# mauriceqch/pcc_geo_cnn_v2

Hardware: AMD Instinct MI355X
Metric: voxel_blocks_64cubed_per_sec_encode_decode (higher is better)
Workload: dtype f32

## Files before the change

include/pcc_geo.h:

```cpp
#ifndef PCC_GEO_H
#define PCC_GEO_H

#include <stddef.h>
#include <stdint.h>

#ifdef __cplusplus
extern "C" {
#endif

#define PCC_ABI_VERSION 4

#define PCC_OK 0
#define PCC_ERR_ARG (-1)
#define PCC_ERR_HIP (-2)
#define PCC_ERR_NOGPU (-3)
#define PCC_ERR_SPACE (-4)
#define PCC_ERR_CORRUPT (-5)

typedef struct pcc_ctx pcc_ctx;

int pcc_abi_version(void);
const char* pcc_last_error(void);
int pcc_ctx_create(int device, pcc_ctx** out);
int pcc_ctx_destroy(pcc_ctx* ctx);
int pcc_ctx_num_cu(pcc_ctx* ctx);

#define PCC_KERNEL_FAMILY 6
#define PCC_NUM_NO_SPLIT 0x1
#define PCC_NUM_NO_SPLIT_DIRECT 0x2
#define PCC_NUM_NO_SPLIT_TR2 0x4
#define PCC_NUM_NO_WINOGRAD 0x8
#define PCC_NUM_NO_WINOGRAD32 0x10
#define PCC_NUM_NO_WINOGRAD64 0x20
#define PCC_NUM_WINO_PER_GROUP 0x40
#define PCC_NUM_NO_TR2M 0x80
#define PCC_NUM_TR2M 0x100
#define PCC_NUM_TR2_OLD 0x200
#define PCC_NUM_SPLIT_MFMA16 0x400
#define PCC_NUM_SPLIT_MFMA32 0x800
#define PCC_NUM_SPLIT_TILE8 0x1000
#define PCC_NUM_P16 0x2000
#define PCC_NUM_NO_F16S 0x4000
#define PCC_NUM_COUT1_T16 0x8000
int pcc_ctx_get_numerics(pcc_ctx* ctx, uint32_t* family, uint32_t* switches);
int pcc_ctx_set_numerics(pcc_ctx* ctx, uint32_t switches);

#define PCC_CONV_BIAS 1
#define PCC_CONV_RELU 2
#define PCC_CONV_ADD 4
#define PCC_CONV_CLIP01 8
#define PCC_CONV_F16 16

#define PCC_CONV_IN16 32
#define PCC_CONV_OUT16 64
#define PCC_CONV_RES16 128

#define PCC_IMPL_AUTO 0
#define PCC_IMPL_GENERIC 1
#define PCC_IMPL_MFMA 2
#define PCC_IMPL_WINOGRAD 3
#define PCC_IMPL_SPLIT 4

typedef struct {
    int32_t N, D, H, W;
    int32_t Cin, Cout;
    int32_t k;
    int32_t stride;
    int32_t transposed;
    int32_t flags;
    int32_t impl;
    int32_t out_cstride;
    int32_t out_coffset;
} pcc_conv_desc;

int pcc_conv_out_dims(const pcc_conv_desc* d, int32_t* OD, int32_t* OH, int32_t* OW);
int pcc_conv_mfma_supported(const pcc_conv_desc* d);
size_t pcc_conv_packed_floats(const pcc_conv_desc* d);
int pcc_conv_pack_weights(const pcc_conv_desc* d, const float* w_keras_host, float* packed_host);
int pcc_conv_kernel_family(pcc_ctx* ctx, const pcc_conv_desc* d, char* buf, int32_t cap);
int pcc_conv3d(pcc_ctx* ctx, const pcc_conv_desc* d, const float* in, const float* w,
               const float* w_packed, const float* bias, const float* residual, float* out,
               void* stream);

#define PCC_NET_ANALYSIS_V1 0
#define PCC_NET_SYNTHESIS_V1 1
#define PCC_NET_ANALYSIS_V2 2
#define PCC_NET_SYNTHESIS_V2 3
#define PCC_NET_ANALYSIS_PROGRESSIVE_V2 4
#define PCC_NET_SYNTHESIS_PROGRESSIVE_V2 5
#define PCC_NET_HYPER_ANALYSIS 6
#define PCC_NET_HYPER_SYNTHESIS 7

int32_t pcc_network_num_layers(int32_t transform, int32_t filters);
int pcc_network_layer(int32_t transform, int32_t filters, int32_t layer, pcc_conv_desc* d, int32_t* residual_role);
size_t pcc_weights_blob_floats(int32_t transform, int32_t filters);
int pcc_weights_pack(int32_t transform, int32_t filters, const float* const* kernels, const float* const* biases,
                     float* blob_host);
int pcc_weights_upload(pcc_ctx* ctx, int32_t transform, int32_t filters, const float* const* kernels,
                       const float* const* biases, float* blob_device, void* stream);
size_t pcc_network_workspace_bytes(int32_t transform, int32_t filters, int32_t N, int32_t D, int32_t H, int32_t W);
int pcc_network_out_dims(int32_t transform, int32_t filters, int32_t D, int32_t H, int32_t W, int32_t* OD, int32_t* OH,
                         int32_t* OW, int32_t* OC);
typedef struct {
    pcc_conv_desc desc;
    int32_t record_amax;
} pcc_layer_plan;
int pcc_network_plan(const pcc_conv_desc* layers, const int32_t* roles, int32_t n, int32_t N, int32_t D, int32_t H, int32_t W,
                     int32_t layer_flags, int32_t final_flags, uint32_t numerics, pcc_layer_plan* plan, int32_t* any_amax);
int pcc_network_forward(pcc_ctx* ctx, int32_t transform, int32_t filters, const float* blob, const float* x, int32_t N,
                        int32_t D, int32_t H, int32_t W, float* y, void* workspace, size_t workspace_bytes,
                        int32_t layer_flags, int32_t final_flags, void* stream);
int pcc_network_forward_analysis(pcc_ctx* ctx, int32_t transform, int32_t filters, const float* blob, const float* x,
                                 int32_t N, int32_t D, int32_t H, int32_t W, float* y, void* workspace,
                                 size_t workspace_bytes, int32_t layer_flags, int32_t final_flags, void* stream);
int pcc_network_forward_synthesis(pcc_ctx* ctx, int32_t transform, int32_t filters, const float* blob, const float* x,
                                  int32_t N, int32_t D, int32_t H, int32_t W, float* y, void* workspace,
                                  size_t workspace_bytes, int32_t layer_flags, int32_t final_flags, void* stream);
int pcc_network_forward_hyper_a(pcc_ctx* ctx, int32_t transform, int32_t filters, const float* blob, const float* x,
                                int32_t N, int32_t D, int32_t H, int32_t W, float* y, void* workspace,
                                size_t workspace_bytes, int32_t layer_flags, int32_t final_flags, void* stream);
int pcc_network_forward_hyper_s(pcc_ctx* ctx, int32_t transform, int32_t filters, const float* blob, const float* x,
                                int32_t N, int32_t D, int32_t H, int32_t W, float* y, void* workspace,
                                size_t workspace_bytes, int32_t layer_flags, int32_t final_flags, void* stream);

typedef struct {
    int32_t version;
    int32_t filters;
    int32_t analysis, synthesis;
    const float* w_analysis;
    const float* w_synthesis;
    const float* w_hyper_analysis;
    const float* w_hyper_synthesis;
// ... 304 lines not shown
```

pcc_geo_cnn_v2_amd/_lib.py:

```python
import ctypes as C
import os

_HERE = os.path.dirname(os.path.abspath(__file__))
LIB_PATH = os.environ.get('PCC_GEO_LIB', os.path.join(_HERE, 'libpcc_geo_hip.so'))

PCC_CONV_BIAS, PCC_CONV_RELU, PCC_CONV_ADD, PCC_CONV_CLIP01, PCC_CONV_F16 = 1, 2, 4, 8, 16
PCC_CONV_IN16, PCC_CONV_OUT16, PCC_CONV_RES16 = 32, 64, 128
PCC_IMPL_AUTO, PCC_IMPL_GENERIC, PCC_IMPL_MFMA, PCC_IMPL_WINOGRAD, PCC_IMPL_SPLIT = 0, 1, 2, 3, 4
PCC_ROUND_FLOOR_HALF, PCC_ROUND_HALF_EVEN = 0, 1
PCC_ANCHOR_NO_CONTEXT, PCC_ANCHOR_HDR_WORDS = 1, 32
PCC_SURFACE_HDR_WORDS = 4
PCC_COLOR_HDR_WORDS = 72

EXPORTS = [
    'pcc_abi_version', 'pcc_last_error', 'pcc_ctx_create', 'pcc_ctx_destroy', 'pcc_ctx_num_cu', 'pcc_ctx_get_numerics', 'pcc_ctx_set_numerics',
    'pcc_conv_out_dims', 'pcc_conv_mfma_supported', 'pcc_conv_packed_floats', 'pcc_conv_pack_weights', 'pcc_conv_kernel_family',
    'pcc_conv3d', 'pcc_quantize', 'pcc_dequantize', 'pcc_scale_to_index', 'pcc_threshold_compact',
    'pcc_threshold_scratch_ints', 'pcc_voxelize', 'pcc_focal_loss', 'pcc_focal_scratch_floats',
    'pcc_symbols_tiles', 'pcc_symbols_pack', 'pcc_symbols_unpack', 'pcc_quantize_pack', 'pcc_index_pack', 'pcc_unpack_dequantize',
    'pcc_range_encode_batch', 'pcc_range_decode_batch', 'pcc_range_encode_batch_n', 'pcc_range_decode_batch_n', 'pcc_pmf_to_quantized_cdf',
    'pcc_d1_search_workspace_bytes', 'pcc_d1_threshold_stats', 'pcc_d12_search_workspace_bytes', 'pcc_d12_threshold_stats', 'pcc_octree_bucket',
    'pcc_d12_search_ties_chunk', 'pcc_d12_search_ties_workspace_bytes', 'pcc_d12_threshold_stats_ties',
    'pcc_network_num_layers', 'pcc_network_layer', 'pcc_weights_blob_floats', 'pcc_weights_pack', 'pcc_weights_upload',
    'pcc_network_workspace_bytes', 'pcc_network_out_dims', 'pcc_network_plan', 'pcc_network_forward', 'pcc_network_forward_analysis',
    'pcc_network_forward_synthesis', 'pcc_network_forward_hyper_a', 'pcc_network_forward_hyper_s',
    'pcc_codec_workspace_bytes', 'pcc_codec_encode', 'pcc_codec_decode_hyper', 'pcc_codec_decode_main',
    'pcc_profile_select', 'pcc_profile_read', 'pcc_normals_workspace_bytes', 'pcc_estimate_normals',
    'pcc_cloud_index_bytes', 'pcc_cloud_index_build', 'pcc_cloud_nearest', 'pcc_cloud_distortion_workspace_bytes', 'pcc_cloud_distortion',
    'pcc_cloud_distortion_ties_workspace_bytes', 'pcc_cloud_distortion_ties',
    'pcc_cloud_map_colors', 'pcc_cloud_color_workspace_bytes', 'pcc_cloud_color_distortion',
    'pcc_cloud_transfer_workspace_bytes', 'pcc_cloud_transfer_colors',
    'pcc_mesh_sample_workspace_bytes', 'pcc_mesh_to_points', 'pcc_render_workspace_bytes', 'pcc_render_points',
    'pcc_conv_wgrad_workspace_bytes', 'pcc_conv_wgrad_slices', 'pcc_conv3d_wgrad', 'pcc_relu_backward', 'pcc_focal_loss_grad', 'pcc_conv_repack_map',
    'pcc_conv_repack_weights_device',
    'pcc_histogram_limits', 'pcc_tensor_histogram_workspace_bytes', 'pcc_tensor_histogram_slices', 'pcc_tensor_histogram', 'pcc_occupancy_scores',
    'pcc_anchor_code_bits', 'pcc_anchor_decode_bits', 'pcc_anchor_encode', 'pcc_anchor_decoder_bytes', 'pcc_anchor_decoder_init',
    'pcc_anchor_decode_level', 'pcc_anchor_decoder_consumed', 'pcc_anchor_tree_capacity', 'pcc_anchor_tree_level_offset',
    'pcc_anchor_tree_workspace_bytes', 'pcc_anchor_tree', 'pcc_anchor_expand_workspace_bytes', 'pcc_anchor_expand', 'pcc_anchor_points',
    'pcc_surface_encode_vertices', 'pcc_surface_decode_vertices', 'pcc_surface_leaves_workspace_bytes', 'pcc_surface_leaves',
    'pcc_surface_edges_workspace_bytes', 'pcc_surface_edges', 'pcc_surface_vertices_workspace_bytes', 'pcc_surface_vertices',
    'pcc_surface_count_workspace_bytes', 'pcc_surface_count', 'pcc_surface_reconstruct_workspace_bytes', 'pcc_surface_reconstruct',
    'pcc_color_anchor_workspace_bytes', 'pcc_color_anchor_plan', 'pcc_color_anchor_forward', 'pcc_color_anchor_inverse',
    'pcc_color_anchor_encode', 'pcc_color_anchor_decode',
    'pcc_rans_stream_cap', 'pcc_rans_workspace_bytes', 'pcc_rans_check_strings', 'pcc_rans_encode_batch', 'pcc_rans_decode_batch',
    'pcc_occ_stream_cap', 'pcc_occ_workspace_bytes', 'pcc_occ_check_strings', 'pcc_occ_encode_batch', 'pcc_occ_decode_batch',
    'pcc_topk_workspace_bytes', 'pcc_topk_compact',
    'pcc_rank_levels_workspace_bytes', 'pcc_rank_levels', 'pcc_d1_count_stats', 'pcc_d12_count_stats',
    'pcc_d1_threshold_stats_hausdorff', 'pcc_d12_threshold_stats_hausdorff', 'pcc_d1_count_stats_hausdorff', 'pcc_d12_count_stats_hausdorff',
    'pcc_quantize_step_pack', 'pcc_index_pack_step', 'pcc_unpack_dequantize_step', 'pcc_rate_ladder',
]
ABI_VERSION = 4
PCC_NUM = dict(no_split=0x1, no_split_direct=0x2, no_split_tr2=0x4, no_winograd=0x8, no_winograd32=0x10, no_winograd64=0x20,
               wino_per_group=0x40, no_tr2m=0x80, tr2m=0x100, tr2_old=0x200, split_mfma16=0x400, split_mfma32=0x800, split_tile8=0x1000,
               p16=0x2000, no_f16s=0x4000, cout1_t16=0x8000)
PCC_ERR_ARG, PCC_ERR_HIP, PCC_ERR_NOGPU, PCC_ERR_SPACE, PCC_ERR_CORRUPT = -1, -2, -3, -4, -5
(PCC_NET_ANALYSIS_V1, PCC_NET_SYNTHESIS_V1, PCC_NET_ANALYSIS_V2, PCC_NET_SYNTHESIS_V2, PCC_NET_ANALYSIS_PROGRESSIVE_V2,
 PCC_NET_SYNTHESIS_PROGRESSIVE_V2, PCC_NET_HYPER_ANALYSIS, PCC_NET_HYPER_SYNTHESIS) = range(8)


class ConvDesc(C.Structure):
    _fields_ = [(n, C.c_int32) for n in ('N', 'D', 'H', 'W', 'Cin', 'Cout', 'k', 'stride', 'transposed',
                                         'flags', 'impl', 'out_cstride', 'out_coffset')]


class LayerPlan(C.Structure):
    _fields_ = [('desc', ConvDesc), ('record_amax', C.c_int32)]


class CdfTable(C.Structure):
    _fields_ = [('cdf', C.POINTER(C.c_int32)), ('cdf_size', C.POINTER(C.c_int32)), ('offset', C.POINTER(C.c_int32)),
                ('rows', C.c_int32), ('cdf_stride', C.c_int32), ('precision', C.c_int32),
                ('overflow_width', C.c_int32)]


class CodecDesc(C.Structure):
    _fields_ = [('version', C.c_int32), ('filters', C.c_int32), ('analysis', C.c_int32), ('synthesis', C.c_int32),
                ('w_analysis', C.c_void_p), ('w_synthesis', C.c_void_p), ('w_hyper_analysis', C.c_void_p),
                ('w_hyper_synthesis', C.c_void_p), ('medians', C.c_void_p), ('scale_table', C.c_void_p),
                ('scale_levels', C.c_int32), ('round_mode', C.c_int32)]


class SymbolSink(C.Structure):
    _fields_ = [('zsym', C.c_void_p), ('ysym', C.c_void_p), ('idx', C.c_void_p), ('zsym_tile_max', C.c_void_p),
                ('ysym_tile_max', C.c_void_p), ('sym_bytes', C.c_int32), ('idx_bytes', C.c_int32), ('channels_first', C.c_int32)]


HISTOGRAM_BUCKETS = 1551


class Histogram(C.Structure):
    _fields_ = [('counts', C.c_uint64 * HISTOGRAM_BUCKETS), ('num', C.c_uint64), ('nonfinite', C.c_uint64), ('min', C.c_double),
                ('max', C.c_double), ('sum', C.c_double), ('sum_squares', C.c_double)]


class Occupancy(C.Structure):
    _fields_ = [(n, C.c_uint64) for n in ('tp', 'tn', 'fp', 'fn', 'num_occupied')]


class PccError(RuntimeError):
    pass


_lib = None


def lib():
    global _lib
    if _lib is not None:
        return _lib
    import torch
    if not os.path.exists(LIB_PATH):
        raise PccError(f'{LIB_PATH} is missing: build it with `make -C pcc_geo_cnn_v2_amd/csrc` '
                       '(python -c "import __graft_entry__ as g; g.build()"). There is no CPU fallback.')
    L = C.CDLL(LIB_PATH)
    vp, i32, sz = C.c_void_p, C.c_int32, C.c_size_t
    L.pcc_abi_version.argtypes, L.pcc_abi_version.restype = [], C.c_int
    L.pcc_last_error.argtypes, L.pcc_last_error.restype = [], C.c_char_p
    L.pcc_ctx_create.argtypes = [C.c_int, C.POINTER(vp)]
    L.pcc_ctx_destroy.argtypes = [vp]
    L.pcc_ctx_num_cu.argtypes = [vp]
    L.pcc_ctx_get_numerics.argtypes = [vp, C.POINTER(C.c_uint32), C.POINTER(C.c_uint32)]
    L.pcc_ctx_set_numerics.argtypes = [vp, C.c_uint32]
    L.pcc_conv_out_dims.argtypes = [C.POINTER(ConvDesc), C.POINTER(i32), C.POINTER(i32), C.POINTER(i32)]
    L.pcc_conv_mfma_supported.argtypes = [C.POINTER(ConvDesc)]
    L.pcc_conv_packed_floats.argtypes = [C.POINTER(ConvDesc)]
    L.pcc_conv_packed_floats.restype = sz
    L.pcc_conv_kernel_family.argtypes = [vp, C.POINTER(ConvDesc), C.c_char_p, i32]
    L.pcc_conv_pack_weights.argtypes = [C.POINTER(ConvDesc), vp, vp]
    L.pcc_conv3d.argtypes = [vp, C.POINTER(ConvDesc), vp, vp, vp, vp, vp, vp, vp]
    L.pcc_quantize.argtypes = [vp, vp, vp, vp, vp, sz, i32, i32, vp]
    L.pcc_dequantize.argtypes = [vp, vp, vp, vp, sz, i32, vp]
    L.pcc_scale_to_index.argtypes = [vp, vp, vp, i32, vp, sz, vp]
    L.pcc_threshold_compact.argtypes = [vp, vp, i32, i32, i32, i32, vp, i32, vp, vp, C.c_int64, vp, vp]
    L.pcc_threshold_scratch_ints.argtypes = [i32, i32, i32, i32]
    L.pcc_threshold_scratch_ints.restype = sz
    L.pcc_voxelize.argtypes = [vp, vp, vp, C.c_int64, i32, i32, i32, i32, vp, vp]
    L.pcc_focal_loss.argtypes = [vp, vp, vp, sz, C.c_float, C.c_float, vp, vp, vp]
    L.pcc_focal_scratch_floats.argtypes, L.pcc_focal_scratch_floats.restype = [], sz
    L.pcc_range_encode_batch.argtypes = [C.POINTER(CdfTable), i32, vp, vp, i32, vp, vp, vp, vp, i32]
    L.pcc_range_decode_batch.argtypes = [C.POINTER(CdfTable), i32, vp, vp, vp, i32, vp, vp, i32]
    L.pcc_range_encode_batch_n.argtypes = [C.POINTER(CdfTable), i32, vp, i32, vp, i32, i32, vp, vp, vp, vp, i32]
    L.pcc_range_decode_batch_n.argtypes = [C.POINTER(CdfTable), i32, vp, vp, vp, i32, i32, vp, vp, i32, i32]
    L.pcc_pmf_to_quantized_cdf.argtypes = [vp, i32, i32, vp]
    L.pcc_d1_search_workspace_bytes.argtypes = [i32, i32, i32, i32]
    L.pcc_d1_search_workspace_bytes.restype = sz
    L.pcc_d1_threshold_stats.argtypes = [vp, vp, i32, i32, i32, i32, vp, i32, i32, vp, vp, C.c_int64, vp, vp, vp, vp, vp, vp]
    L.pcc_d12_search_workspace_bytes.argtypes = [i32, i32, i32, i32, C.c_int64]
    L.pcc_d12_search_workspace_bytes.restype = sz
    L.pcc_d12_threshold_stats.argtypes = [vp, vp, i32, i32, i32, i32, vp, i32, i32, vp, vp, vp, C.c_int64, vp, vp, vp, vp, vp, vp, vp, vp, vp, vp]
    L.pcc_d12_search_ties_chunk.argtypes = [i32, i32, i32, i32]
    L.pcc_d12_search_ties_chunk.restype = i32
    L.pcc_d12_search_ties_workspace_bytes.argtypes = [i32, i32, i32, i32, C.c_int64, C.c_int64]
    L.pcc_d12_search_ties_workspace_bytes.restype = sz
    L.pcc_d12_threshold_stats_ties.argtypes = [vp, vp, i32, i32, i32, i32, vp, i32, i32, vp, vp, vp, C.c_int64, vp, C.c_int64, vp, vp, vp, vp, vp, vp,
                                               vp, vp, vp, vp]
    L.pcc_normals_workspace_bytes.argtypes = [C.c_int64, i32]
    L.pcc_normals_workspace_bytes.restype = sz
    L.pcc_estimate_normals.argtypes = [vp, vp, C.c_int64, i32, vp, vp, vp, vp, vp]
    L.pcc_cloud_index_bytes.argtypes = [C.c_int64]
    L.pcc_cloud_index_bytes.restype = sz
    L.pcc_cloud_index_build.argtypes = [vp, vp, C.c_int64, vp, vp]
    L.pcc_cloud_nearest.argtypes = [vp, vp, C.c_int64, vp, C.c_int64, vp, vp, vp]
    L.pcc_cloud_distortion_workspace_bytes.argtypes = [C.c_int64, C.c_int64]
    L.pcc_cloud_distortion_workspace_bytes.restype = sz
    L.pcc_cloud_distortion.argtypes = [vp, vp, C.c_int64, vp, C.c_int64, vp, vp, vp, vp, vp, vp]
    L.pcc_cloud_distortion_ties_workspace_bytes.argtypes = [C.c_int64, C.c_int64, i32, C.c_int64]
    L.pcc_cloud_distortion_ties_workspace_bytes.restype = sz
    L.pcc_cloud_distortion_ties.argtypes = [vp, vp, C.c_int64, vp, C.c_int64, vp, i32, C.c_int64, vp, vp, vp, vp, vp, vp]
    L.pcc_cloud_map_colors.argtypes = [vp, vp, C.c_int64, vp, vp, C.c_int64, i32, vp, vp, vp]
    L.pcc_cloud_color_workspace_bytes.argtypes = [C.c_int64, C.c_int64]
    L.pcc_cloud_color_workspace_bytes.restype = sz
    L.pcc_cloud_color_distortion.argtypes = [vp, vp, C.c_int64, vp, vp, C.c_int64, vp, vp, vp, vp]
    L.pcc_cloud_transfer_workspace_bytes.argtypes = [C.c_int64, C.c_int64]
    L.pcc_cloud_transfer_workspace_bytes.restype = sz
    L.pcc_cloud_transfer_colors.argtypes = [vp, vp, C.c_int64, vp, vp, C.c_int64, vp, vp, vp, vp]
    L.pcc_mesh_sample_workspace_bytes.argtypes = [C.c_int64, C.c_int64]
    L.pcc_mesh_sample_workspace_bytes.restype = sz
    L.pcc_mesh_to_points.argtypes = [vp, vp, C.c_int64, vp, C.c_int64, C.c_int64, C.c_uint64, i32, vp, vp, vp, vp, vp]
    L.pcc_render_workspace_bytes.argtypes = [i32, i32]
    L.pcc_render_workspace_bytes.restype = sz
# ... 124 lines not shown
```

pcc_geo_cnn_v2_amd/csrc/common.h:

```cpp
#pragma once
#include <hip/hip_runtime.h>

#include <cstdarg>
#include <cstdio>

#include "../../include/pcc_geo.h"

struct pcc_ctx {
    int device;
    int num_cu;
    hipDeviceProp_t prop;
    void* profile = nullptr;
    void* scratch = nullptr;
    size_t scratch_bytes = 0;
    uint32_t numerics = 0;
    bool num(uint32_t bit) const { return (numerics & bit) != 0; }
    unsigned* amax = nullptr;
    int amax_cap = 0;
    void* summary_limits = nullptr;
};
int pcc_ctx_amax(pcc_ctx* ctx, int n, unsigned** ptr);
constexpr int PCC_AMAX_SLOTS = 64;
struct pcc_conv_ext { const unsigned* in_amax; unsigned* out_amax; bool out_recorded; };
#ifdef __HIPCC__
// ... 64 lines not shown
}
int pcc_conv3d_ext(pcc_ctx* ctx, const pcc_conv_desc* d, const float* in, const float* w, const float* w_packed, const float* bias,
                   const float* residual, float* out, pcc_conv_ext* ext, void* stream);
uint32_t* pcc_threshold_mask_of(int32_t* scratch, int32_t B, int32_t D);
int pcc_threshold_from_mask(pcc_ctx* ctx, int32_t B, int32_t D, int32_t H, int32_t W, float* xyz, int32_t* counts, int64_t cap,
                            int32_t* scratch, hipStream_t st);
bool pcc_wino_eligible(const pcc_conv_desc* d);
int pcc_conv_wino(pcc_ctx* ctx, const pcc_conv_desc* d, const float* in, const float* u_packed,
                  const float* bias, const float* residual, float* out, hipStream_t st);
bool pcc_tr2m_eligible(const pcc_conv_desc* d);
int pcc_conv_tr2m(pcc_ctx* ctx, const pcc_conv_desc* d, const float* in, const float* w_tr2g, const float* bias, float* out,
                  hipStream_t st);
size_t pcc_tr2m_bf16_packed_floats(int Cin, int Cout);
void pcc_tr2m_bf16_pack(int Cin, int Cout, const float* w_tr2g, float* out);
bool pcc_tr2m_bf16_covers(const pcc_conv_desc* d);
int pcc_conv_tr2m_bf16(pcc_ctx* ctx, const pcc_conv_desc* d, const float* in, const float* w_split, const float* bias, float* out,
                       pcc_conv_ext* ext, hipStream_t st);
constexpr int PCC_TR2M_F16S_TAIL = 64;
size_t pcc_tr2m_f16s_packed_floats(int Cin, int Cout);
void pcc_tr2m_f16s_pack(int Cin, int Cout, const float* w_tr2g, float* out);
int pcc_conv_tr2m_f16s(pcc_ctx* ctx, const pcc_conv_desc* d, const float* in, const float* w_f16s, const float* bias, float* out,
                       pcc_conv_ext* ext, hipStream_t st);
bool pcc_tr2m_f16_covers(const pcc_conv_desc* d);
int pcc_conv_tr2m_f16(pcc_ctx* ctx, const pcc_conv_desc* d, const float* in, const float* w_tr2g, const float* bias, void* out,
                      hipStream_t st);
bool pcc_f16_eligible(const pcc_conv_desc* d);
size_t pcc_f16_packed_bytes(int C);
void pcc_f16_pack(int C, const float* wlog, unsigned short* out);
int pcc_conv_f16(pcc_ctx* ctx, const pcc_conv_desc* d, const void* in, const void* w_packed, const float* bias,
                 const void* residual, void* out, bool out32, hipStream_t st);
constexpr int PCC_WINO_U_FLOATS = 48 * 64 * 4;
constexpr int PCC_WINO_UB_FLOATS = 48 * 2 * 64 * 4;
void pcc_wino_bf16_pack(int ngroups, const float* u_f32, float* out);
int pcc_conv_wino_bf16(pcc_ctx* ctx, const pcc_conv_desc* d, const float* in, const float* ub_packed, const float* bias,
                       const float* residual, float* out, hipStream_t st);
constexpr int PCC_WINO_UH_FLOATS = 64 * 776 / 4;
constexpr int PCC_WINO_UH_TAIL = 64;
bool pcc_wino_f16s_covers(const pcc_conv_desc* d);
void pcc_wino_f16s_pack(int ngroups, const float* u_f32, float* out);
int pcc_conv_wino_f16s(pcc_ctx* ctx, const pcc_conv_desc* d, const float* in, const float* uh_packed, const float* bias,
                       const float* residual, float* out, pcc_conv_ext* ext, hipStream_t st);
size_t pcc_split_packed_floats(int C);
void pcc_split_pack(int C, const float* wlog, float* out);
bool pcc_split_covers(const pcc_conv_desc* d);
bool pcc_tr2_split_covers(const pcc_conv_desc* d);
int pcc_conv_tr2_split(pcc_ctx* ctx, const pcc_conv_desc* d, const float* in, const float* w_split, const float* bias, float* out,
                       pcc_conv_ext* ext, hipStream_t st);
int pcc_conv_split(pcc_ctx* ctx, const pcc_conv_desc* d, bool mfma32, const float* in, const float* w_split, const float* bias,
                   const float* residual, float* out, hipStream_t st);
int pcc_conv_fwd(pcc_ctx* ctx, const pcc_conv_desc* d, const float* in, const float* w_packed, const float* bias, const float* residual,
                 float* out, int tx, hipStream_t st);
int pcc_conv_tr2(pcc_ctx* ctx, const pcc_conv_desc* d, const float* in, const float* w_packed, const float* bias, const float* residual,
                 float* out, int tx, hipStream_t st);
int pcc_conv_cin1(pcc_ctx* ctx, const pcc_conv_desc* d, const float* in, const float* w_packed, const float* bias, const float* residual,
                  float* out, pcc_conv_ext* ext, hipStream_t st);
int pcc_conv_cout1_mfma(pcc_ctx* ctx, const pcc_conv_desc* d, const float* in, const float* w_packed, const float* bias,
                        const float* residual, float* out, const pcc_thr_fuse* fuse, bool* fused, hipStream_t st);
int pcc_conv_cout1(pcc_ctx* ctx, const pcc_conv_desc* d, const float* in, const float* w_packed, const float* bias, const float* residual,
                   float* out, hipStream_t st);
#include <utility>
#include <vector>
inline int pcc_enable_big_lds(const void* kern, int lds_bytes) {
    if (lds_bytes <= 64 * 1024) return PCC_OK;
    static thread_local std::vector<std::pair<const void*, int>> done;
    int dev = 0;
    PCC_CHECK_HIP(hipGetDevice(&dev));
    for (const auto& e : done)
        if (e.first == kern && e.second == dev) return PCC_OK;
    PCC_CHECK_HIP(hipFuncSetAttribute(kern, hipFuncAttributeMaxDynamicSharedMemorySize, lds_bytes));
    done.emplace_back(kern, dev);
    return PCC_OK;
}

inline bool pcc_wino_channels(int cin, int cout) { return cin == cout && (cin == 16 || cin == 32 || cin == 64); }
```

pcc_geo_cnn_v2_amd/csrc/conv_route.hip:

```cpp
#include <cstdlib>

#include "common.h"

namespace {

enum Kind { K_NONE = 0, K_FWD, K_TR2, K_CIN1, K_COUT1, K_COUT1M };

struct Plan {
    Kind kind = K_NONE;
    int tx = 0;
    bool flip = false;
};

inline int base_w(const pcc_conv_desc* d) {
    if (d->transposed) return d->W;
    return pcc_same_out(d->W, d->stride);
}

static Plan make_plan(const pcc_conv_desc* d) {
    Plan p;
    if ((double)d->D * d->H * d->W * d->Cin * 4.0 >= 2147483648.0) return p;
    const bool out_vec_ok = d->out_cstride == 0 || (d->out_cstride % 4 == 0 && d->out_coffset % 4 == 0);
    const int k = d->k, s = d->stride;
    const bool even = (d->D % 2 == 0) && (d->H % 2 == 0) && (d->W % 2 == 0);
// ... 185 lines not shown
    PCC_REQUIRE(p.kind != K_NONE, "pcc_conv_pack_weights: shape not covered by the MFMA path");
    const Packed L = packed_layout(d, p.kind);
    const Taps Wf{d, w, p.flip};
    switch (p.kind) {
        case K_FWD: return pack_fwd(d, Wf, L, pk);
        case K_TR2: pack_tr2(d, Wf, L, pk); break;
        case K_CIN1: pack_cin1(d, Wf, pk); break;
        case K_COUT1M: pack_cout1m(Wf, pk); break;
        default: pack_cout1(d, Wf, pk);
    }
    return PCC_OK;
}

pcc_conv_family pcc_conv_route(const pcc_conv_desc* d, uint32_t numerics) {
    auto num = [numerics](uint32_t bits) { return (numerics & bits) != 0; };
    const Plan p = make_plan(d);
    const int ci = d->Cin, fl = d->flags, impl = d->impl;
    const bool autoi = impl == PCC_IMPL_AUTO;
    if (p.kind == K_NONE || !(autoi || impl == PCC_IMPL_MFMA || impl == PCC_IMPL_WINOGRAD || impl == PCC_IMPL_SPLIT)) return PCC_FAM_GENERIC;
    if ((fl & (PCC_CONV_IN16 | PCC_CONV_RES16)) && p.kind != K_COUT1M) return PCC_FAM_F16;
    if (p.kind == K_CIN1) return PCC_FAM_CIN1;
    if (p.kind == K_COUT1M) return PCC_FAM_COUT1M;
    if (p.kind == K_COUT1) return PCC_FAM_COUT1;
    const bool plain = !(fl & (PCC_CONV_F16 | PCC_CONV_OUT16));
    if (p.kind == K_TR2) {
        if (d->k != 3) return PCC_FAM_TR2;
        if (autoi && !num(PCC_NUM_NO_TR2M) && pcc_tr2m_f16_covers(d)) return PCC_FAM_TR2M_F16;
        const bool f16s = plain && !num(PCC_NUM_NO_TR2M | PCC_NUM_NO_SPLIT | PCC_NUM_NO_SPLIT_TR2 | PCC_NUM_NO_F16S) && pcc_tr2m_eligible(d);
        if (autoi && f16s) return PCC_FAM_TR2M_F16S;
        if (autoi && plain && pcc_tr2_split_covers(d) && !num(PCC_NUM_NO_SPLIT | PCC_NUM_NO_SPLIT_TR2)) return PCC_FAM_TR2_SPLIT;
        if (num(PCC_NUM_NO_TR2M) || !pcc_tr2m_eligible(d) || !(num(PCC_NUM_TR2M) || ci == 32 || d->D >= 32)) return PCC_FAM_TR2;
        if (f16s) return PCC_FAM_TR2M_F16S;
        return pcc_tr2m_bf16_covers(d) && !num(PCC_NUM_NO_SPLIT | PCC_NUM_NO_SPLIT_TR2) ? PCC_FAM_TR2M_BF16 : PCC_FAM_TR2M;
    }
    const pcc_conv_family fwd = (fl & PCC_CONV_F16) ? PCC_FAM_FWD_F16 : PCC_FAM_FWD;
    if (!(pcc_wino_channels(ci, d->Cout) && d->k == 3 && d->stride == 1)) return fwd;
    const bool mfma32 = !num(PCC_NUM_SPLIT_MFMA16) && (num(PCC_NUM_SPLIT_MFMA32) || ci == 32) && (d->W % 32 == 0 || d->W == 16);
    const pcc_conv_family split = mfma32 ? PCC_FAM_SPLIT32 : PCC_FAM_SPLIT16;
    if (impl == PCC_IMPL_SPLIT) return split;
    if (autoi && ci == 64 && !(fl & (PCC_CONV_F16 | PCC_CONV_OUT16 | PCC_CONV_CLIP01)) &&
        !num(PCC_NUM_NO_SPLIT | PCC_NUM_NO_F16S | PCC_NUM_NO_WINOGRAD | PCC_NUM_NO_WINOGRAD64) && pcc_wino_eligible(d))
        return PCC_FAM_WINO_F16S;
    if (autoi && plain && !num(PCC_NUM_NO_SPLIT | PCC_NUM_NO_SPLIT_DIRECT) && pcc_split_covers(d) &&
        (ci == 64 || (ci == 32 && d->D <= 16 && (d->W % 32 == 0 || d->W == 16))))
        return split;
    const bool want = impl == PCC_IMPL_WINOGRAD || (autoi && !(fl & PCC_CONV_F16) && !num(PCC_NUM_NO_WINOGRAD) &&
                                                    !(ci == 32 && (num(PCC_NUM_NO_WINOGRAD32) || d->D < 16)) && !(ci == 64 && num(PCC_NUM_NO_WINOGRAD64)));
    if (!(want && pcc_wino_eligible(d))) return fwd;
    if (!num(PCC_NUM_NO_SPLIT | PCC_NUM_NO_F16S) && (ci == 16 || !(fl & PCC_CONV_CLIP01)) && !(ci == 64 && (fl & PCC_CONV_F16))) return PCC_FAM_WINO_F16S;
    if (!num(PCC_NUM_NO_SPLIT) && ci == 16) return PCC_FAM_WINO_BF16;
    return PCC_FAM_WINO;
}

PCC_API int pcc_conv_kernel_family(pcc_ctx* ctx, const pcc_conv_desc* d, char* buf, int32_t cap) {
    PCC_REQUIRE(ctx && d && buf && cap > 0, "pcc_conv_kernel_family: NULL argument");
    static const char* const names[PCC_FAM_COUNT] = {
        "generic (reference-order fp32 FMA chain)", "conv_f16 (fp16 storage, f16 MFMA)", "conv_fwd (exact fp32 MFMA)", "conv_fwd (f16 MFMA)",
        "conv_k3s1_split (direct, bf16 x 3, 16x16x32 MFMA)", "conv_k3s1_split32 (direct, bf16 x 3, 32x32x16 MFMA)",
        "conv16_wino (Winograd, exact fp32 MFMA)", "conv16_wino_bf16 (Winograd, bf16 x 3)", "conv16_wino_f16s (Winograd, fp16 x 2 under a per-block pre-scale)",
        "conv_tr2 (exact fp32 MFMA)", "conv_tr2m_f16 (z march, f16 MFMA)", "conv_tr2m_f16s (z march, fp16 x 2 under a per-block pre-scale)",
        "conv_tr2_split (parity classes, bf16 x 3)", "conv_tr2m_bf16 (z march, bf16 x 3)", "conv_tr2m (z march, exact fp32 MFMA)",
        "conv_cin1 (exact fp32 MFMA)", "conv_cout1_mfma (exact fp32 MFMA)", "conv_cout1 (fp32 VALU)"};
    snprintf(buf, (size_t)cap, "%s", names[pcc_conv_route(d, ctx->numerics)]);
    return PCC_OK;
}

int pcc_conv3d_mfma_thr(pcc_ctx* ctx, const pcc_conv_desc* d, const float* in, const float* w_packed, const float* bias,
                        const float* residual, float* out, const pcc_thr_fuse* fuse, bool* fused, pcc_conv_ext* ext, hipStream_t st) {
    if (fused) *fused = false;
    if (ext) ext->out_recorded = false;
    const Plan p = make_plan(d);
    const pcc_conv_family fam = pcc_conv_route(d, ctx->numerics);
    PCC_REQUIRE(fam != PCC_FAM_GENERIC, "pcc_conv3d_mfma: shape not covered");
    const Packed L = packed_layout(d, p.kind);
    PCC_REQUIRE(!(d->flags & PCC_CONV_OUT16) || p.kind == K_FWD || p.kind == K_TR2 || p.kind == K_CIN1,
                "pcc_conv3d: PCC_CONV_OUT16 needs a layer with Cout a multiple of 16");
    PCC_REQUIRE(!(d->flags & PCC_CONV_OUT16) || d->impl != PCC_IMPL_WINOGRAD, "pcc_conv3d: PCC_CONV_OUT16 is not implemented by the Winograd kernel (fp32)");
    switch (fam) {
        case PCC_FAM_F16:
            PCC_REQUIRE(p.kind == K_FWD && (d->flags & PCC_CONV_IN16) && pcc_f16_eligible(d),
                        "pcc_conv3d: PCC_CONV_IN16 covers k3 stride-1 layers with Cin = Cout in {16, 32, 64} (H, W multiples of 16) and the 16 -> 1 transposed layer");
            return pcc_conv_f16(ctx, d, in, w_packed + L.f16, bias, residual, out, !(d->flags & PCC_CONV_OUT16), st);
        case PCC_FAM_SPLIT16:
        case PCC_FAM_SPLIT32:
            PCC_REQUIRE(d->Cin >= 32 && pcc_split_covers(d) && !(d->flags & (PCC_CONV_F16 | PCC_CONV_OUT16)), "pcc_conv3d: PCC_IMPL_SPLIT covers fp32 k3 stride-1 layers with Cin = Cout in {32, 64}, W % 16 == 0");
            return pcc_conv_split(ctx, d, fam == PCC_FAM_SPLIT32, in, w_packed + L.split, bias, residual, out, st);
        case PCC_FAM_WINO_F16S: return pcc_conv_wino_f16s(ctx, d, in, w_packed + L.wino_uh, bias, residual, out, ext, st);
        case PCC_FAM_WINO_BF16: return pcc_conv_wino_bf16(ctx, d, in, w_packed + L.wino_ub, bias, residual, out, st);
        case PCC_FAM_WINO: return pcc_conv_wino(ctx, d, in, w_packed + L.wino_u, bias, residual, out, st);
        case PCC_FAM_FWD:
        case PCC_FAM_FWD_F16:
            PCC_REQUIRE(d->impl != PCC_IMPL_WINOGRAD, "%s", L.wino_u ? "pcc_conv3d: PCC_IMPL_WINOGRAD needs W and H multiples of 16"
                                                                     : "pcc_conv3d: PCC_IMPL_WINOGRAD covers Cin = Cout in {16,32,64} k3 stride-1 layers only");
            return pcc_conv_fwd(ctx, d, in, w_packed, bias, residual, out, p.tx, st);
        case PCC_FAM_TR2M_F16: return pcc_conv_tr2m_f16(ctx, d, in, w_packed + L.tr2g, bias, out, st);
        case PCC_FAM_TR2M_F16S: return pcc_conv_tr2m_f16s(ctx, d, in, w_packed + L.tr2_f16s, bias, out, ext, st);
        case PCC_FAM_TR2_SPLIT: return pcc_conv_tr2_split(ctx, d, in, w_packed + L.tr2_split, bias, out, ext, st);
        case PCC_FAM_TR2M_BF16: return pcc_conv_tr2m_bf16(ctx, d, in, w_packed + L.tr2_split, bias, out, ext, st);
        case PCC_FAM_TR2M: return pcc_conv_tr2m(ctx, d, in, w_packed + L.tr2g, bias, out, st);
        case PCC_FAM_TR2: return pcc_conv_tr2(ctx, d, in, w_packed, bias, residual, out, p.tx, st);
        case PCC_FAM_CIN1: return pcc_conv_cin1(ctx, d, in, w_packed, bias, residual, out, ext, st);
        case PCC_FAM_COUT1M: return pcc_conv_cout1_mfma(ctx, d, in, w_packed, bias, residual, out, fuse, fused, st);
        case PCC_FAM_COUT1: return pcc_conv_cout1(ctx, d, in, w_packed, bias, residual, out, st);
        default: break;
    }
    pcc_set_error("pcc_conv3d_mfma: no kernel for family %d", (int)fam);
    return PCC_ERR_ARG;
}

PCC_API int pcc_conv_repack_map(const pcc_conv_desc* d, int32_t* map) {
    PCC_REQUIRE(d && map, "pcc_conv_repack_map: NULL argument");
    const Plan p = make_plan(d);
    PCC_REQUIRE(p.kind != K_NONE, "pcc_conv_repack_map: shape not covered by the MFMA path");
    const Packed L = packed_layout(d, p.kind);
    const size_t taps = (size_t)d->k * d->k * d->k * d->Cin * d->Cout;
    PCC_REQUIRE(taps < (size_t(1) << 24), "pcc_conv_repack_map: kernel too large for an fp32 iota");
    size_t base_end = L.total;
    for (size_t off : {L.wino_u, L.f16, L.wino_ub, L.split, L.wino_uh, L.tr2g, L.tr2_split, L.tr2_f16s})
        if (off && off < base_end) base_end = off;
    float* iota = (float*)malloc(taps * sizeof(float));
    float* pk = (float*)malloc(L.total * sizeof(float));
    if (!iota || !pk) { free(iota); free(pk); PCC_REQUIRE(false, "pcc_conv_repack_map: out of memory"); }
    for (size_t i = 0; i < taps; ++i) iota[i] = (float)(i + 1);
    const int rc = pcc_conv_pack_weights(d, iota, pk);
    if (rc == PCC_OK)
        for (size_t i = 0; i < L.total; ++i) {
            const bool gathered = i < base_end || (L.tr2g && i >= L.tr2g && i < L.tr2g + (size_t)27 * d->Cin * d->Cout);
            map[i] = gathered ? (int32_t)pk[i] - 1 : -2;
        }
    free(iota);
    free(pk);
    return rc;
}
```

pcc_geo_cnn_v2_amd/csrc/ctx.hip:

```cpp
#include <cstring>
#include <new>

#include <cstdlib>

#include "common.h"

static thread_local char g_err[512] = "";

void pcc_set_error(const char* fmt, ...) {
    va_list ap;
    va_start(ap, fmt);
    vsnprintf(g_err, sizeof(g_err), fmt, ap);
    va_end(ap);
}

PCC_API int pcc_abi_version(void) { return PCC_ABI_VERSION; }
PCC_API const char* pcc_last_error(void) { return g_err; }

PCC_API int pcc_ctx_create(int device, pcc_ctx** out) {
    PCC_REQUIRE(out != nullptr, "pcc_ctx_create: out is NULL");
    int n = 0;
    if (hipGetDeviceCount(&n) != hipSuccess || n <= 0) {
        pcc_set_error("pcc_ctx_create: no HIP device visible");
        return PCC_ERR_NOGPU;
    }
    PCC_REQUIRE(device >= 0 && device < n, "pcc_ctx_create: device %d out of range [0,%d)", device, n);
    pcc_ctx* c = new (std::nothrow) pcc_ctx();
    PCC_REQUIRE(c != nullptr, "pcc_ctx_create: out of memory");
    c->device = device;
    hipError_t e = hipGetDeviceProperties(&c->prop, device);
    if (e != hipSuccess) {
        delete c;
        pcc_set_error("hipGetDeviceProperties failed: %s", hipGetErrorString(e));
        return PCC_ERR_HIP;
    }
    if (strncmp(c->prop.gcnArchName, "gfx950", 6) != 0) {
        pcc_set_error("pcc_ctx_create: device %d is %s, this library is built for gfx950 only", device,
                      c->prop.gcnArchName);
        delete c;
        return PCC_ERR_NOGPU;
    }
    c->num_cu = c->prop.multiProcessorCount;
    c->numerics = pcc_numerics_from_env();
    *out = c;
    return PCC_OK;
}

uint32_t pcc_numerics_from_env() {
    static const struct { const char* name; uint32_t bit; } flags[] = {
        {"PCC_NO_SPLIT", PCC_NUM_NO_SPLIT}, {"PCC_NO_SPLIT_DIRECT", PCC_NUM_NO_SPLIT_DIRECT}, {"PCC_NO_SPLIT_TR2", PCC_NUM_NO_SPLIT_TR2},
        {"PCC_NO_WINOGRAD", PCC_NUM_NO_WINOGRAD}, {"PCC_NO_WINOGRAD32", PCC_NUM_NO_WINOGRAD32}, {"PCC_NO_WINOGRAD64", PCC_NUM_NO_WINOGRAD64},
        {"PCC_WINO_PER_GROUP", PCC_NUM_WINO_PER_GROUP}, {"PCC_NO_TR2M", PCC_NUM_NO_TR2M}, {"PCC_TR2M", PCC_NUM_TR2M},
        {"PCC_TR2_OLD", PCC_NUM_TR2_OLD}, {"PCC_NO_F16S", PCC_NUM_NO_F16S}, {"PCC_COUT1_T16", PCC_NUM_COUT1_T16}};
    uint32_t m = 0;
    for (const auto& f : flags)
        if (getenv(f.name) != nullptr) m |= f.bit;
    if (const char* v = getenv("PCC_SPLIT_MFMA")) m |= atoi(v) == 16 ? PCC_NUM_SPLIT_MFMA16 : atoi(v) == 32 ? PCC_NUM_SPLIT_MFMA32 : 0u;
    if (const char* v = getenv("PCC_SPLIT_TILE")) m |= atoi(v) == 8 ? PCC_NUM_SPLIT_TILE8 : 0u;
    if (const char* v = getenv("PCC_P16")) m |= atoi(v) ? PCC_NUM_P16 : 0u;
    return m;
}

PCC_API int pcc_ctx_get_numerics(pcc_ctx* ctx, uint32_t* family, uint32_t* switches) {
    PCC_REQUIRE(ctx != nullptr, "pcc_ctx_get_numerics: ctx is NULL");
    if (family) *family = PCC_KERNEL_FAMILY;
    if (switches) *switches = ctx->numerics;
    return PCC_OK;
}

PCC_API int pcc_ctx_set_numerics(pcc_ctx* ctx, uint32_t switches) {
    PCC_REQUIRE(ctx != nullptr, "pcc_ctx_set_numerics: ctx is NULL");
    PCC_REQUIRE((switches & ~0xffffu) == 0, "pcc_ctx_set_numerics: unknown bits 0x%x", switches & ~0xffffu);
    ctx->numerics = switches;
    return PCC_OK;
}

int pcc_ctx_scratch(pcc_ctx* ctx, size_t bytes, void** ptr) {
    if (bytes > ctx->scratch_bytes) {
        if (ctx->scratch) PCC_CHECK_HIP(hipFree(ctx->scratch));
        ctx->scratch = nullptr; ctx->scratch_bytes = 0;
        PCC_CHECK_HIP(hipMalloc(&ctx->scratch, bytes));
        ctx->scratch_bytes = bytes;
    }
    *ptr = ctx->scratch;
    return PCC_OK;
}

int pcc_ctx_amax(pcc_ctx* ctx, int n, unsigned** ptr) {
    if (n > ctx->amax_cap) {
        if (ctx->amax) PCC_CHECK_HIP(hipFree(ctx->amax));
        ctx->amax = nullptr; ctx->amax_cap = 0;
        const int cap = n > 4096 ? n : 4096;
        PCC_CHECK_HIP(hipMalloc((void**)&ctx->amax, (size_t)cap * sizeof(unsigned)));
        ctx->amax_cap = cap;
    }
    *ptr = ctx->amax;
    return PCC_OK;
}

PCC_API int pcc_ctx_destroy(pcc_ctx* ctx) {
    if (ctx) pcc_profile_free(ctx);
    if (ctx) pcc_rans_free(ctx);
    if (ctx && ctx->scratch) (void)hipFree(ctx->scratch);
    if (ctx && ctx->amax) (void)hipFree(ctx->amax);
    if (ctx && ctx->summary_limits) (void)hipFree(ctx->summary_limits);
    delete ctx;
    return PCC_OK;
}

PCC_API int pcc_ctx_num_cu(pcc_ctx* ctx) {
    PCC_REQUIRE(ctx != nullptr, "pcc_ctx_num_cu: ctx is NULL");
    return ctx->num_cu;
}

PCC_API int pcc_conv_out_dims(const pcc_conv_desc* d, int32_t* OD, int32_t* OH, int32_t* OW) {
    PCC_REQUIRE(d && OD && OH && OW, "pcc_conv_out_dims: NULL argument");
    PCC_REQUIRE(d->stride >= 1, "pcc_conv_out_dims: stride must be >= 1");
    if (d->transposed) {
        *OD = d->D * d->stride; *OH = d->H * d->stride; *OW = d->W * d->stride;
    } else {
        *OD = pcc_same_out(d->D, d->stride); *OH = pcc_same_out(d->H, d->stride); *OW = pcc_same_out(d->W, d->stride);
    }
    return PCC_OK;
}

// ... 39 lines not shown
```

Before: 8510.

## Add z-marching MFMA kernel for stride-2 Cin16→Cout32 forward conv

Adds a dedicated forward conv kernel for stride-2, k3, Cin16/Cout32 fp32 layers. Each block walks along z and keeps a 5-plane LDS ring of input planes plus all weights in LDS. The next two planes are prefetched with buffer-to-LDS loads that are interleaved with the MFMA chain, so each plane is loaded once and reused across the kz taps. The z-split adapts to the CU count. It is routed by default when shapes fit, and an env/numerics switch can turn it off. The cost is high LDS use (one block per CU) and a new code path for these layers.

```diff
diff --git a/include/pcc_geo.h b/include/pcc_geo.h
--- a/include/pcc_geo.h
+++ b/include/pcc_geo.h
@@ -42,6 +42,7 @@
 #define PCC_NUM_P16 0x2000
 #define PCC_NUM_NO_F16S 0x4000
 #define PCC_NUM_COUT1_T16 0x8000
+#define PCC_NUM_NO_FWD_MARCH 0x10000
 int pcc_ctx_get_numerics(pcc_ctx* ctx, uint32_t* family, uint32_t* switches);
 int pcc_ctx_set_numerics(pcc_ctx* ctx, uint32_t switches);
 
@@ -78,6 +79,7 @@
 size_t pcc_conv_packed_floats(const pcc_conv_desc* d);
 int pcc_conv_pack_weights(const pcc_conv_desc* d, const float* w_keras_host, float* packed_host);
 int pcc_conv_kernel_family(pcc_ctx* ctx, const pcc_conv_desc* d, char* buf, int32_t cap);
+int pcc_conv_fwd_marches(const pcc_conv_desc* d, uint32_t numerics);
 int pcc_conv3d(pcc_ctx* ctx, const pcc_conv_desc* d, const float* in, const float* w,
                const float* w_packed, const float* bias, const float* residual, float* out,
                void* stream);
diff --git a/pcc_geo_cnn_v2_amd/_lib.py b/pcc_geo_cnn_v2_amd/_lib.py
--- a/pcc_geo_cnn_v2_amd/_lib.py
+++ b/pcc_geo_cnn_v2_amd/_lib.py
@@ -48,11 +48,12 @@
     'pcc_rank_levels_workspace_bytes', 'pcc_rank_levels', 'pcc_d1_count_stats', 'pcc_d12_count_stats',
     'pcc_d1_threshold_stats_hausdorff', 'pcc_d12_threshold_stats_hausdorff', 'pcc_d1_count_stats_hausdorff', 'pcc_d12_count_stats_hausdorff',
     'pcc_quantize_step_pack', 'pcc_index_pack_step', 'pcc_unpack_dequantize_step', 'pcc_rate_ladder',
+    'pcc_conv_fwd_marches',
 ]
 ABI_VERSION = 4
 PCC_NUM = dict(no_split=0x1, no_split_direct=0x2, no_split_tr2=0x4, no_winograd=0x8, no_winograd32=0x10, no_winograd64=0x20,
                wino_per_group=0x40, no_tr2m=0x80, tr2m=0x100, tr2_old=0x200, split_mfma16=0x400, split_mfma32=0x800, split_tile8=0x1000,
-               p16=0x2000, no_f16s=0x4000, cout1_t16=0x8000)
+               p16=0x2000, no_f16s=0x4000, cout1_t16=0x8000, no_fwd_march=0x10000)
 PCC_ERR_ARG, PCC_ERR_HIP, PCC_ERR_NOGPU, PCC_ERR_SPACE, PCC_ERR_CORRUPT = -1, -2, -3, -4, -5
 (PCC_NET_ANALYSIS_V1, PCC_NET_SYNTHESIS_V1, PCC_NET_ANALYSIS_V2, PCC_NET_SYNTHESIS_V2, PCC_NET_ANALYSIS_PROGRESSIVE_V2,
  PCC_NET_SYNTHESIS_PROGRESSIVE_V2, PCC_NET_HYPER_ANALYSIS, PCC_NET_HYPER_SYNTHESIS) = range(8)
@@ -126,6 +127,7 @@
     L.pcc_conv_packed_floats.argtypes = [C.POINTER(ConvDesc)]
     L.pcc_conv_packed_floats.restype = sz
     L.pcc_conv_kernel_family.argtypes = [vp, C.POINTER(ConvDesc), C.c_char_p, i32]
+    L.pcc_conv_fwd_marches.argtypes = [C.POINTER(ConvDesc), C.c_uint32]
     L.pcc_conv_pack_weights.argtypes = [C.POINTER(ConvDesc), vp, vp]
     L.pcc_conv3d.argtypes = [vp, C.POINTER(ConvDesc), vp, vp, vp, vp, vp, vp, vp]
     L.pcc_quantize.argtypes = [vp, vp, vp, vp, vp, sz, i32, i32, vp]
diff --git a/pcc_geo_cnn_v2_amd/csrc/common.h b/pcc_geo_cnn_v2_amd/csrc/common.h
--- a/pcc_geo_cnn_v2_amd/csrc/common.h
+++ b/pcc_geo_cnn_v2_amd/csrc/common.h
@@ -140,6 +140,10 @@
                  float* out, int tx, hipStream_t st);
 int pcc_conv_tr2(pcc_ctx* ctx, const pcc_conv_desc* d, const float* in, const float* w_packed, const float* bias, const float* residual,
                  float* out, int tx, hipStream_t st);
+bool pcc_fwd_march_covers(const pcc_conv_desc* d);
+bool pcc_fwd_march_route(const pcc_conv_desc* d, uint32_t numerics);
+int pcc_conv_fwd_march(pcc_ctx* ctx, const pcc_conv_desc* d, const float* in, const float* w_packed, const float* bias,
+                       const float* residual, float* out, hipStream_t st);
 int pcc_conv_cin1(pcc_ctx* ctx, const pcc_conv_desc* d, const float* in, const float* w_packed, const float* bias, const float* residual,
                   float* out, pcc_conv_ext* ext, hipStream_t st);
 int pcc_conv_cout1_mfma(pcc_ctx* ctx, const pcc_conv_desc* d, const float* in, const float* w_packed, const float* bias,
diff --git a/pcc_geo_cnn_v2_amd/csrc/conv_fwd_march.hip b/pcc_geo_cnn_v2_amd/csrc/conv_fwd_march.hip
--- /dev/null
+++ b/pcc_geo_cnn_v2_amd/csrc/conv_fwd_march.hip
@@ -0,0 +1,201 @@
+#include "conv_direct.h"
+
+namespace pccfwdm {
+
+using namespace pcck;
+using namespace pccmfma;
+
+constexpr int NT = 256, NWAVE = 4, NRING = 5;
+constexpr int CIN = 16, COUT = 32, NCT = 2;
+constexpr int NFRAG = 27 * NCT;
+
+template <int TX_>
+struct MarchCfg {
+    static constexpr int TX = TX_;
+    static constexpr int RY = 16 / TX, TY = NWAVE * RY;
+    static constexpr int LY = 2 * TY + 1, LX = 2 * TX + 1;
+    static constexpr int NV = LY * LX;
+    static constexpr int SLOTS = NV * 4;
+    static constexpr int ITEMS = (SLOTS + NT - 1) / NT;
+    static constexpr int PLANE_BYTES = NWAVE * ITEMS * 1024;
+    static constexpr int W_BASE = NRING * PLANE_BYTES;
+    static constexpr int LDS_BYTES = W_BASE + NFRAG * 1024;
+    static_assert(16 % TX == 0 && 2 * ITEMS <= 27, "bad tile");
+    static_assert(LDS_BYTES <= 160 * 1024, "LDS budget");
+};
+
+template <int TX>
+__global__ void __launch_bounds__(NT, 1) conv_fwd_march_kernel(ConvArgs a, int zlen) {
+    using C = MarchCfg<TX>;
+    extern __shared__ __attribute__((aligned(16))) unsigned char smem[];
+    typedef __attribute__((address_space(3))) void* lds_ptr;
+    auto ldsr = [&](unsigned off) -> f32x4 { return *reinterpret_cast<const f32x4*>(smem + off); };
+    const int tid = threadIdx.x, lane = tid & 63, wave = __builtin_amdgcn_readfirstlane(tid >> 6);
+    const int v = lane & 15, cq = lane >> 4;
+
+    int t = xcd_remap(blockIdx.x, gridDim.x);
+    const int tx = t % a.ntx; t /= a.ntx;
+    const int ty = t % a.nty; t /= a.nty;
+    const int zs = t % a.ntz;
+    const int n = t / a.ntz;
+    const int oz0 = zs * zlen, oy0 = ty * C::TY, ox0 = tx * TX;
+    const int iy0 = 2 * oy0, ix0 = 2 * ox0;
+
+    const size_t HW = (size_t)a.H * a.W;
+    const unsigned HWI = (unsigned)(HW * CIN * 4);
+    const float* in_n = a.in + (size_t)n * a.D * HW * CIN;
+
+    {
+        const __amdgpu_buffer_rsrc_t rw = make_rsrc(a.w, (unsigned)NFRAG * 1024u);
+        for (int p = wave; p < NFRAG; p += NWAVE)
+            __builtin_amdgcn_raw_ptr_buffer_load_lds(rw, (lds_ptr)(smem + C::W_BASE + p * 1024), 16, lane * 16, p * 1024, 0, 0);
+    }
+    unsigned rel[C::ITEMS];
+#pragma unroll
+    for (int it = 0; it < C::ITEMS; ++it) {
+        const int slot = (wave * C::ITEMS + it) * 64 + lane;
+        const int u = slot >> 2, q = slot & 3;
+        const int ly = u / C::LX, lx = u - ly * C::LX;
+        const int gy = iy0 + ly, gx = ix0 + lx;
+        const bool ok = slot < C::SLOTS && gy < a.H && gx < a.W;
+        rel[it] = ok ? (unsigned)((((gy * a.W + gx) * CIN) + q * 4) * 4) : kOOB;
+    }
+    auto stage = [&](unsigned ring_off, int plane) __attribute__((always_inline)) {
+        const bool ok = plane < a.D;
+        const __amdgpu_buffer_rsrc_t rp = make_rsrc(ok ? in_n + (size_t)plane * HW * CIN : in_n, ok ? HWI : 0u);
+#pragma unroll
+        for (int it = 0; it < C::ITEMS; ++it)
+            __builtin_amdgcn_raw_ptr_buffer_load_lds(rp, (lds_ptr)(smem + ring_off + (wave * C::ITEMS + it) * 1024), 16, (int)rel[it], 0, 0, 0);
+    };
+
+    const int ry = v / TX, rx = v % TX;
+    const int oyl = wave * C::RY + ry;
+    const unsigned lane_b = (unsigned)(((2 * oyl) * C::LX + 2 * rx) * 64 + cq * 16);
+    const unsigned lane_w = (unsigned)(C::W_BASE + lane * 16);
+
+    const int pz0 = 2 * oz0;
+#pragma unroll
+    for (int k = 0; k < 3; ++k) stage((unsigned)(k * C::PLANE_BYTES), pz0 + k);
+    __builtin_amdgcn_s_waitcnt(0x0F70);
+    __syncthreads();
+
+    const bool has_res = (a.flags & PCC_CONV_ADD) != 0;
+    const f32x4 zero4 = {0.f, 0.f, 0.f, 0.f};
+    f32x4 bias4[NCT];
+#pragma unroll
+    for (int ct = 0; ct < NCT; ++ct)
+        bias4[ct] = (a.flags & PCC_CONV_BIAS) ? *reinterpret_cast<const f32x4*>(a.bias + ct * 16 + cq * 4) : zero4;
+
+    int s0 = 0;
+#pragma unroll 1
+    for (int j = 0; j < zlen; ++j) {
+        const size_t vox = (((size_t)n * a.OD + (oz0 + j)) * a.OH + (oy0 + oyl)) * a.OW + (ox0 + rx);
+        f32x4 resv[NCT];
+#pragma unroll
+        for (int ct = 0; ct < NCT; ++ct)
+            resv[ct] = has_res ? *reinterpret_cast<const f32x4*>(a.res + vox * COUT + ct * 16 + cq * 4) : zero4;
+
+        unsigned bofs[3];
+#pragma unroll
+        for (int kz = 0; kz < 3; ++kz) {
+            int s = s0 + kz;
+            s = s >= NRING ? s - NRING : s;
+            bofs[kz] = lane_b + (unsigned)(s * C::PLANE_BYTES);
+        }
+        const int pnext = pz0 + 2 * j + 3;
+        const bool ok0 = j + 1 < zlen && pnext < a.D, ok1 = j + 1 < zlen && pnext + 1 < a.D;
+        const __amdgpu_buffer_rsrc_t rnext0 = make_rsrc(ok0 ? in_n + (size_t)pnext * HW * CIN : in_n, ok0 ? HWI : 0u);
+        const __amdgpu_buffer_rsrc_t rnext1 = make_rsrc(ok1 ? in_n + (size_t)(pnext + 1) * HW * CIN : in_n, ok1 ? HWI : 0u);
+        unsigned onext[2];
+#pragma unroll
+        for (int k = 0; k < 2; ++k) {
+            int s = s0 + 3 + k;
+            s = s >= NRING ? s - NRING : s;
+            onext[k] = (unsigned)(s * C::PLANE_BYTES + wave * C::ITEMS * 1024);
+        }
+        f32x4 acc[NCT];
+#pragma unroll
+        for (int ct = 0; ct < NCT; ++ct) acc[ct] = zero4;
+        f32x4 bb[2], wf[2][NCT];
+        bb[0] = ldsr(bofs[0]);
+#pragma unroll
+        for (int ct = 0; ct < NCT; ++ct) wf[0][ct] = ldsr(lane_w + (unsigned)(ct * 1024));
+#pragma unroll
+        for (int q = 0; q < 27; ++q) {
+            if (q + 1 < 27) {
+                const int tn = q + 1;
+                bb[tn & 1] = ldsr(bofs[tn / 9] + (unsigned)((((tn / 3) % 3) * C::LX + tn % 3) * 64));
+#pragma unroll
+                for (int ct = 0; ct < NCT; ++ct) wf[tn & 1][ct] = ldsr(lane_w + (unsigned)((tn * NCT + ct) * 1024));
+            }
+            __builtin_amdgcn_sched_barrier(0);
+#pragma unroll
+            for (int jj = 0; jj < 4; ++jj) {
+#pragma unroll
+                for (int ct = 0; ct < NCT; ++ct) acc[ct] = mfma16(wf[q & 1][ct][jj], bb[q & 1][jj], acc[ct]);
+                if (jj == 1 && q < C::ITEMS)
+                    __builtin_amdgcn_raw_ptr_buffer_load_lds(rnext0, (lds_ptr)(smem + onext[0] + q * 1024), 16, (int)rel[q], 0, 0, 0);
+                if (jj == 1 && q >= C::ITEMS && q < 2 * C::ITEMS)
+                    __builtin_amdgcn_raw_ptr_buffer_load_lds(rnext1, (lds_ptr)(smem + onext[1] + (q - C::ITEMS) * 1024), 16, (int)rel[q - C::ITEMS], 0, 0, 0);
+            }
+            PCC_PIN_MEM_MFMA();
+        }
+        __builtin_amdgcn_s_waitcnt(0x0F70);
+        __syncthreads();
+        s0 += 2;
+        s0 = s0 >= NRING ? s0 - NRING : s0;
+#pragma unroll
+        for (int ct = 0; ct < NCT; ++ct) {
+            f32x4 o = acc[ct];
+            if (a.flags & PCC_CONV_BIAS) o += bias4[ct];
+            if (a.flags & PCC_CONV_RELU) { o.x = fmaxf(o.x, 0.f); o.y = fmaxf(o.y, 0.f); o.z = fmaxf(o.z, 0.f); o.w = fmaxf(o.w, 0.f); }
+            if (has_res) o += resv[ct];
+            if (a.flags & PCC_CONV_CLIP01) {
+                o.x = fminf(fmaxf(o.x, 0.f), 1.f); o.y = fminf(fmaxf(o.y, 0.f), 1.f);
+                o.z = fminf(fmaxf(o.z, 0.f), 1.f); o.w = fminf(fmaxf(o.w, 0.f), 1.f);
+            }
+            *reinterpret_cast<f32x4*>(a.out + vox * a.ocs + a.oco + ct * 16 + cq * 4) = o;
+        }
+    }
+}
+
+static int march_tx(const pcc_conv_desc* d) {
+    if (d->transposed || d->k != 3 || d->stride != 2 || d->Cin != CIN || d->Cout != COUT) return 0;
+    if (d->flags & (PCC_CONV_F16 | PCC_CONV_OUT16 | PCC_CONV_IN16 | PCC_CONV_RES16)) return 0;
+    if ((d->D | d->H | d->W) & 1) return 0;
+    const int ocs = d->out_cstride ? d->out_cstride : d->Cout;
+    if (ocs % 4 || d->out_coffset % 4) return 0;
+    if ((double)d->D * d->H * d->W * d->Cin * 4.0 >= 2147483648.0) return 0;
+    const int oh = d->H / 2, ow = d->W / 2;
+    if (ow % 16 == 0 && oh % MarchCfg<16>::TY == 0) return 16;
+    if (ow % 8 == 0 && oh % MarchCfg<8>::TY == 0) return 8;
+    return 0;
+}
+
+template <int TX>
+static int launch_march(const pcc_ctx* ctx, ConvArgs a, hipStream_t st) {
+    using C = MarchCfg<TX>;
+    a.nty = a.OH / C::TY; a.ntx = a.OW / TX;
+    const int base = a.N * a.nty * a.ntx;
+    int zsplit = 1;
+    while (base * zsplit < ctx->num_cu && a.OD % (zsplit * 2) == 0 && a.OD / (zsplit * 2) >= 2) zsplit *= 2;
+    a.ntz = zsplit;
+    return launch(conv_fwd_march_kernel<TX>, NT, C::LDS_BYTES, base * zsplit, a, st, a.OD / zsplit);
+}
+
+}
+
+using namespace pccfwdm;
+
+bool pcc_fwd_march_covers(const pcc_conv_desc* d) { return march_tx(d) != 0; }
+
+int pcc_conv_fwd_march(pcc_ctx* ctx, const pcc_conv_desc* d, const float* in, const float* w_packed, const float* bias,
+                       const float* residual, float* out, hipStream_t st) {
+    const ConvArgs a = conv_args(d, in, w_packed, bias, residual, out);
+    switch (march_tx(d)) {
+        case 16: return launch_march<16>(ctx, a, st);
+        case 8: return launch_march<8>(ctx, a, st);
+        default: break;
+    }
+    return no_instantiation(d);
+}
diff --git a/pcc_geo_cnn_v2_amd/csrc/conv_route.hip b/pcc_geo_cnn_v2_amd/csrc/conv_route.hip
--- a/pcc_geo_cnn_v2_amd/csrc/conv_route.hip
+++ b/pcc_geo_cnn_v2_amd/csrc/conv_route.hip
@@ -261,6 +261,16 @@
     return PCC_FAM_WINO;
 }
 
+bool pcc_fwd_march_route(const pcc_conv_desc* d, uint32_t numerics) {
+    if (numerics & PCC_NUM_NO_FWD_MARCH) return false;
+    return pcc_conv_route(d, numerics) == PCC_FAM_FWD && pcc_fwd_march_covers(d);
+}
+
+PCC_API int pcc_conv_fwd_marches(const pcc_conv_desc* d, uint32_t numerics) {
+    PCC_REQUIRE(d, "pcc_conv_fwd_marches: NULL argument");
+    return pcc_fwd_march_route(d, numerics) ? 1 : 0;
+}
+
 PCC_API int pcc_conv_kernel_family(pcc_ctx* ctx, const pcc_conv_desc* d, char* buf, int32_t cap) {
     PCC_REQUIRE(ctx && d && buf && cap > 0, "pcc_conv_kernel_family: NULL argument");
     static const char* const names[PCC_FAM_COUNT] = {
@@ -301,6 +311,7 @@
         case PCC_FAM_FWD_F16:
             PCC_REQUIRE(d->impl != PCC_IMPL_WINOGRAD, "%s", L.wino_u ? "pcc_conv3d: PCC_IMPL_WINOGRAD needs W and H multiples of 16"
                                                                      : "pcc_conv3d: PCC_IMPL_WINOGRAD covers Cin = Cout in {16,32,64} k3 stride-1 layers only");
+            if (fam == PCC_FAM_FWD && pcc_fwd_march_route(d, ctx->numerics)) return pcc_conv_fwd_march(ctx, d, in, w_packed, bias, residual, out, st);
             return pcc_conv_fwd(ctx, d, in, w_packed, bias, residual, out, p.tx, st);
         case PCC_FAM_TR2M_F16: return pcc_conv_tr2m_f16(ctx, d, in, w_packed + L.tr2g, bias, out, st);
         case PCC_FAM_TR2M_F16S: return pcc_conv_tr2m_f16s(ctx, d, in, w_packed + L.tr2_f16s, bias, out, ext, st);
diff --git a/pcc_geo_cnn_v2_amd/csrc/ctx.hip b/pcc_geo_cnn_v2_amd/csrc/ctx.hip
--- a/pcc_geo_cnn_v2_amd/csrc/ctx.hip
+++ b/pcc_geo_cnn_v2_amd/csrc/ctx.hip
@@ -51,7 +51,8 @@
         {"PCC_NO_SPLIT", PCC_NUM_NO_SPLIT}, {"PCC_NO_SPLIT_DIRECT", PCC_NUM_NO_SPLIT_DIRECT}, {"PCC_NO_SPLIT_TR2", PCC_NUM_NO_SPLIT_TR2},
         {"PCC_NO_WINOGRAD", PCC_NUM_NO_WINOGRAD}, {"PCC_NO_WINOGRAD32", PCC_NUM_NO_WINOGRAD32}, {"PCC_NO_WINOGRAD64", PCC_NUM_NO_WINOGRAD64},
         {"PCC_WINO_PER_GROUP", PCC_NUM_WINO_PER_GROUP}, {"PCC_NO_TR2M", PCC_NUM_NO_TR2M}, {"PCC_TR2M", PCC_NUM_TR2M},
-        {"PCC_TR2_OLD", PCC_NUM_TR2_OLD}, {"PCC_NO_F16S", PCC_NUM_NO_F16S}, {"PCC_COUT1_T16", PCC_NUM_COUT1_T16}};
+        {"PCC_TR2_OLD", PCC_NUM_TR2_OLD}, {"PCC_NO_F16S", PCC_NUM_NO_F16S}, {"PCC_COUT1_T16", PCC_NUM_COUT1_T16},
+        {"PCC_NO_FWD_MARCH", PCC_NUM_NO_FWD_MARCH}};
     uint32_t m = 0;
     for (const auto& f : flags)
         if (getenv(f.name) != nullptr) m |= f.bit;
@@ -70,7 +71,7 @@
 
 PCC_API int pcc_ctx_set_numerics(pcc_ctx* ctx, uint32_t switches) {
     PCC_REQUIRE(ctx != nullptr, "pcc_ctx_set_numerics: ctx is NULL");
-    PCC_REQUIRE((switches & ~0xffffu) == 0, "pcc_ctx_set_numerics: unknown bits 0x%x", switches & ~0xffffu);
+    PCC_REQUIRE((switches & ~0x1ffffu) == 0, "pcc_ctx_set_numerics: unknown bits 0x%x", switches & ~0x1ffffu);
     ctx->numerics = switches;
     return PCC_OK;
 }
```

After: 8502 (median of 2 runs). No clear change (-0.1%).
